# IntuitionMachines/volta

Hardware: AMD Instinct MI355X
Metric: image-text pairs/sec, ctrl_vilbert_base pretrain step (higher is better)
Workload: dtype bf16

## Files before the change

include/volta_hip.h:

```cpp
#ifndef VOLTA_HIP_H
#define VOLTA_HIP_H
#include <stddef.h>
#include <stdint.h>

#ifdef __cplusplus
extern "C" {
#endif

typedef void* vk_stream_t;

int vk_version(void);
const char* vk_device_arch(void);
const char* vk_last_error(void);

typedef struct vk_dropout {
    const uint64_t* seed;
    uint32_t site;
    uint32_t threshold;
    float scale;
} vk_dropout;

int vk_set_seed(uint64_t* seed_dev, uint64_t seed, vk_stream_t s);

int vk_cast_f32_bf16(const float* src, void* dst, int64_t n, vk_stream_t s);
// ... 256 lines not shown
int vk_nce_negatives(vk_dropout rng, int B, int R, int32_t* out, vk_stream_t s);

enum { VK_TASK_BCE_SCALED = 0, VK_TASK_BCE_MEAN = 1, VK_TASK_BCE_REGIONS = 2, VK_TASK_CE_OPTIONS = 3 };
typedef struct vk_task_loss_args {
    const float* logits;
    const void* target;
    const int64_t* mask;
    void* work;
    float* out;
    int32_t* row_argmax;
    int32_t kind, groups, n, ld;
} vk_task_loss_args;
int64_t vk_task_loss_work_bytes(int groups);
int vk_task_loss_fwd(const vk_task_loss_args* a, vk_stream_t s);
int vk_task_loss_bwd(const vk_task_loss_args* a, const float* gscale, void* dlogits, vk_stream_t s);

int vk_mask_prep(const int64_t* mask, float* out, int n, vk_stream_t s);

#define VK_CHUNK_SKIP 255
int vk_grad_norm_workspace_floats(void);
int vk_grad_norm_clip(const float* g, int64_t n, float pre_scale, float max_norm, float* partial, float* out, vk_stream_t s);
int vk_grad_norm_clip_masked(const float* g, int64_t n, const uint8_t* chunk_class, float pre_scale, float max_norm, float* partial, float* out, vk_stream_t s);
int vk_grad_sqnorm_chunks(const float* g, int64_t chunk0, int64_t nchunks, const uint8_t* chunk_class, float* sums, vk_stream_t s);
int vk_grad_norm_from_chunks(float* sums, int64_t total_chunks, float pre_scale, float max_norm, float* out, vk_stream_t s);
typedef struct vk_adamw_args {
    float* p;
    const float* g;
    float* m;
    float* v;
    void* shadow;
    const uint8_t* chunk_class;
    const float* clip;
    int64_t n;
    float cls_lr_mult[8];
    float cls_wd[8];
    float lr, beta1, beta2, eps, step_mult, grad_scale;
} vk_adamw_args;
int vk_adamw_step(const vk_adamw_args* a, vk_stream_t s);
int vk_adamw_step_on(const vk_adamw_args* a, int ncus, vk_stream_t s);
typedef struct vk_adamw_tensor {
    float* p;
    const float* g;
    float* m;
    float* v;
    int64_t numel;
    int32_t cls;
// ... 23 lines not shown
int vk_radam_step_list(const vk_radam_args* a, const vk_adamw_tensor* list, int n, int64_t max_numel, vk_stream_t s);
int vk_axpy_f32(float* y, const float* x, float alpha, int64_t n, vk_stream_t s);
int vk_sum_slabs_f32(float* dst, const float* src, int64_t slab_stride, int nslabs, int64_t n, vk_stream_t s);
int vk_sum_slabs_bf16(void* dst, const float* src, int64_t slab_stride, int nslabs, int64_t n, const int32_t* dyn_rows, int row_len, vk_stream_t s);
int vk_memset_async(void* p, int value, int64_t bytes, vk_stream_t s);
int vk_hold_cus(int nwg, int usec, int whole_cu, vk_stream_t s);
int vk_gate_wait(const uint64_t* flag, const uint64_t* stamp, int timeout_us, int32_t* err, vk_stream_t s);
int vk_bump_u64(uint64_t* word, vk_stream_t s);
int vk_store_u64(uint64_t* word, uint64_t value, vk_stream_t s);
int vk_gate_value(const uint64_t* flag, uint64_t want, int timeout_us, int32_t* err, vk_stream_t s);
int vk_comm_standin(const void* src, void* dst, int64_t bytes, int nwg, int min_usec, uint64_t* stamps, vk_stream_t s);
int vk_gemm_reserve_cus(int n);
#define VK_TAIL_MAX_JOBS 16
typedef struct vk_tail_job {
    float* dst;
    float* dst2;
    const float* src;
    const float* src2;
    int64_t stride;
    int64_t n;
    int32_t kind, count;
    int32_t accumulate;
    int32_t block_start;
} vk_tail_job;
int vk_side_tail(const vk_tail_job* jobs, int njobs, vk_stream_t s);

int vk_mul_bf16(const void* a, const void* b, void* out, int64_t n, const int32_t* dyn_rows, int row_len, vk_stream_t s);

enum {
    VK_OP_GEMM = 1,
    VK_OP_LN_FWD, VK_OP_LN_BWD,
    VK_OP_ATTN_FWD,
    VK_OP_ATTN_BWD,
    VK_OP_EMBED_FWD, VK_OP_EMBED_BWD, VK_OP_XENT_FWD,
    VK_OP_XENT_BWD,
    VK_OP_KL_FWD, VK_OP_KL_BWD,
    VK_OP_GENERIC,
    VK_OP_SIDE_BEGIN, VK_OP_SIDE_END, VK_OP_WAIT_SIDE, VK_OP_JOIN,
    VK_OP_LN_FINALIZE,
    VK_OP_GEMM_FP8,
    VK_OP_GEMM_CHAIN
};
enum {
    VK_FN_CAST = 1, VK_FN_MEMSET, VK_FN_LOC_FWD, VK_FN_LOC_BWD, VK_FN_ADD_DROPOUT, VK_FN_COLSUM, VK_FN_SELECT,
    VK_FN_GATHER, VK_FN_SCATTER_ADD, VK_FN_LOSS_FINAL, VK_FN_POOL_FWD, VK_FN_POOL_BWD, VK_FN_MASK_PREP, VK_FN_MUL,
    VK_FN_VLBERT_PREP, VK_FN_VLBERT_MASKGRAD, VK_FN_ROWGROUP_SUM, VK_FN_RELU_BWD, VK_FN_COPY, VK_FN_SUM_SLABS, VK_FN_SUM_SLABS_BF16,
// ... 103 lines not shown
```

volta_amd/_lib.py:

```python
import ctypes as C
import os

import torch

_HERE = os.path.dirname(os.path.abspath(__file__))
LIB_PATH = os.path.join(_HERE, "libvolta_hip_%s.so" % os.environ["VK_LIB"] if os.environ.get("VK_LIB") else "libvolta_hip.so")
GEMM_PERSISTENT, GEMM_ONE_TILE_PER_WG, GEMM_SOFT_START = 0x1000, 0x2000, 0x4000


class VoltaHipError(RuntimeError):
    pass


if not os.path.exists(LIB_PATH):
    raise ImportError(
        "volta_amd: %s not found. The HIP kernels are the product; there is no fallback path. "
        "Build with `make -C volta_amd/csrc` (hipcc --offload-arch=gfx950)." % LIB_PATH)

lib = C.CDLL(LIB_PATH)

c_p = C.c_void_p
i32 = C.c_int32
CHUNK_SKIP = 255

# ... 112 lines not shown
class RadamArgs(C.Structure):
    _fields_ = [("p", c_p), ("g", c_p), ("m", c_p), ("v", c_p), ("shadow", c_p), ("chunk_class", c_p), ("clip", c_p),
                ("n", C.c_int64), ("cls_decay", C.c_float * RADAM_CLASSES), ("cls_step", C.c_float * RADAM_CLASSES),
                ("cls_rect", i32 * RADAM_CLASSES), ("beta1", C.c_float), ("beta2", C.c_float), ("one_minus_beta1", C.c_float),
                ("one_minus_beta2", C.c_float), ("eps", C.c_float), ("grad_scale", C.c_float)]


class GradSeedArgs(C.Structure):
    _fields_ = [("src", c_p), ("stride_b", C.c_int64), ("stride_l", C.c_int64), ("dst", c_p), ("y", c_p), ("B", i32), ("L", i32), ("H", i32),
                ("row0", i32), ("ld", i32), ("ldy", i32), ("accumulate", i32), ("reserved_", i32)]


PAIR_MAX_SEGS = 8


class PairGatherArgs(C.Structure):
    _fields_ = [("src", c_p * PAIR_MAX_SEGS), ("dst", c_p * PAIR_MAX_SEGS), ("bytes", C.c_int64 * PAIR_MAX_SEGS), ("side", i32 * PAIR_MAX_SEGS),
                ("cap_idx", c_p), ("img_idx", c_p), ("n_items", C.c_int64 * 2), ("nseg", i32), ("npairs", i32), ("c0", i32), ("nc", i32),
                ("i0", i32), ("ni", i32)]


class TailJob(C.Structure):
    _fields_ = [("dst", c_p), ("dst2", c_p), ("src", c_p), ("src2", c_p), ("stride", C.c_int64), ("n", C.c_int64), ("kind", i32), ("count", i32),
                ("accumulate", i32), ("block_start", i32)]


TAIL_MAX_JOBS = 16


class GenericArgs(C.Structure):
    _fields_ = [("fn", i32), ("p", c_p * 6), ("n", C.c_int64 * 6), ("f", C.c_float * 2), ("drop", Dropout)]


class Op(C.Structure):
    _fields_ = [("kind", i32), ("i0", i32), ("i1", i32), ("i2", i32), ("a", c_p), ("b", c_p), ("c", c_p)]


(OP_GEMM, OP_LN_FWD, OP_LN_BWD, OP_ATTN_FWD, OP_ATTN_BWD, OP_EMBED_FWD, OP_EMBED_BWD, OP_XENT_FWD, OP_XENT_BWD,
 OP_KL_FWD, OP_KL_BWD, OP_GENERIC, OP_SIDE_BEGIN, OP_SIDE_END, OP_WAIT_SIDE, OP_JOIN, OP_LN_FINALIZE, OP_GEMM_FP8, OP_GEMM_CHAIN) = range(1, 20)
(FN_CAST, FN_MEMSET, FN_LOC_FWD, FN_LOC_BWD, FN_ADD_DROPOUT, FN_COLSUM, FN_SELECT, FN_GATHER, FN_SCATTER_ADD,
 FN_LOSS_FINAL, FN_POOL_FWD, FN_POOL_BWD, FN_MASK_PREP, FN_MUL, FN_VLBERT_PREP, FN_VLBERT_MASKGRAD, FN_ROWGROUP_SUM,
 FN_RELU_BWD, FN_COPY, FN_SUM_SLABS, FN_SUM_SLABS_BF16, FN_SIDE_TAIL, FN_QUANT_ROWS, FN_CAST_FP8, FN_VIS_LOSS_FWD, FN_VIS_LOSS_BWD,
 FN_NCE_NEG, FN_TEXT_END_ROWS, FN_VLBERT_OBJ_IDS, FN_VLBERT_POSITIONS, FN_HOLD, FN_GATE, FN_BUMP, FN_GRAD_SEED) = range(1, 35)


class AttnArgs(C.Structure):
    _fields_ = [("q", c_p * 2), ("k", c_p * 2), ("v", c_p * 2), ("ld", i32 * 2), ("L", i32 * 2), ("mask", c_p * 2),
# ... 78 lines not shown
_sig("vk_vlbert_positions", C.c_int, c_p, C.c_int, C.c_int, C.c_int, c_p, c_p, c_p)
_sig("vk_vis_loss_fwd", C.c_int, C.POINTER(VisLossArgs), c_p)
_sig("vk_vis_loss_bwd", C.c_int, C.POINTER(VisLossArgs), c_p, C.c_int, c_p, c_p)
_sig("vk_task_loss_work_bytes", C.c_int64, C.c_int)
_sig("vk_task_loss_fwd", C.c_int, C.POINTER(TaskLossArgs), c_p)
_sig("vk_task_loss_bwd", C.c_int, C.POINTER(TaskLossArgs), c_p, c_p, c_p)
_sig("vk_nce_negatives", C.c_int, Dropout, C.c_int, C.c_int, c_p, c_p)
_sig("vk_pool_mul_bwd", C.c_int, c_p, C.c_int, c_p, c_p, c_p, c_p, C.c_int, C.c_int, Dropout, c_p)
_sig("vk_mask_prep", C.c_int, c_p, c_p, C.c_int, c_p)
_sig("vk_mul_bf16", C.c_int, c_p, c_p, c_p, C.c_int64, c_p, C.c_int, c_p)
_sig("vk_grad_norm_workspace_floats", C.c_int)
_sig("vk_grad_norm_clip", C.c_int, c_p, C.c_int64, C.c_float, C.c_float, c_p, c_p, c_p)
_sig("vk_adamw_step", C.c_int, C.POINTER(AdamwArgs), c_p)
_sig("vk_adamw_step_on", C.c_int, C.POINTER(AdamwArgs), C.c_int, c_p)
_sig("vk_grad_norm_clip_masked", C.c_int, c_p, C.c_int64, c_p, C.c_float, C.c_float, c_p, c_p, c_p)
_sig("vk_adamw_step_list", C.c_int, C.POINTER(AdamwArgs), c_p, C.c_int, C.c_int64, c_p)
_sig("vk_grad_sqnorm_list", C.c_int, c_p, C.c_int, C.c_int64, c_p, c_p, c_p)
_sig("vk_grad_sqnorm_list_work_floats", C.c_int)
_sig("vk_grad_seed", C.c_int, C.POINTER(GradSeedArgs), c_p)
_sig("vk_pair_gather", C.c_int, C.POINTER(PairGatherArgs), c_p)
_sig("vk_radam_step", C.c_int, C.POINTER(RadamArgs), c_p)
_sig("vk_radam_step_list", C.c_int, C.POINTER(RadamArgs), c_p, C.c_int, C.c_int64, c_p)
_sig("vk_grad_sqnorm_chunks", C.c_int, c_p, C.c_int64, C.c_int64, c_p, c_p, c_p)
_sig("vk_grad_norm_from_chunks", C.c_int, c_p, C.c_int64, C.c_float, C.c_float, c_p, c_p)
_sig("vk_axpy_f32", C.c_int, c_p, c_p, C.c_float, C.c_int64, c_p)
_sig("vk_sum_slabs_f32", C.c_int, c_p, c_p, C.c_int64, C.c_int, C.c_int64, c_p)
_sig("vk_sum_slabs_bf16", C.c_int, c_p, c_p, C.c_int64, C.c_int, C.c_int64, c_p, C.c_int, c_p)
_sig("vk_memset_async", C.c_int, c_p, C.c_int, C.c_int64, c_p)
_sig("vk_hold_cus", C.c_int, C.c_int, C.c_int, C.c_int, c_p)
_sig("vk_gate_wait", C.c_int, c_p, c_p, C.c_int, c_p, c_p)
_sig("vk_bump_u64", C.c_int, c_p, c_p)
_sig("vk_store_u64", C.c_int, c_p, C.c_uint64, c_p)
_sig("vk_gate_value", C.c_int, c_p, C.c_uint64, C.c_int, c_p, c_p)
_sig("vk_comm_standin", C.c_int, c_p, c_p, C.c_int64, C.c_int, C.c_int, c_p, c_p)
_sig("vk_gemm_reserve_cus", C.c_int, C.c_int)
_sig("vk_side_tail", C.c_int, C.POINTER(TailJob), C.c_int, c_p)
_sig("vk_run_ops", C.c_int, C.POINTER(Op), C.c_int, c_p)
_sig("vk_run_ops_timed", C.c_int, C.POINTER(Op), C.c_int, c_p, C.POINTER(C.c_float))
_sig("vk_ln_bwd_finalize", C.c_int, C.POINTER(LnBwdArgs), c_p)
_sig("vk_ln_fwd_pair", C.c_int, C.POINTER(LnArgs), C.POINTER(LnArgs), c_p)
_sig("vk_ln_bwd_pair", C.c_int, C.POINTER(LnBwdArgs), C.POINTER(LnBwdArgs), c_p)
_sig("vk_concap_batch", C.c_int, C.POINTER(ConcapArgs), c_p)
_sig("vk_side_join", C.c_int, c_p)
_sig("vk_side_join_from", C.c_int, c_p, c_p)
_sig("vk_side_enable", None, C.c_int)
_sig("vk_side_stream", c_p, c_p)

EXPORTS = ["vk_version", "vk_device_arch", "vk_last_error", "vk_set_seed", "vk_cast_f32_bf16", "vk_gemm_grouped", "vk_gemm_grouped_ex", "vk_gemm_chain", "vk_gemm_split_workspace_bytes", "vk_gemm_fp8_grouped", "vk_quant_rows_fp8", "vk_cast_bf16_fp8",
           "vk_ln_fwd", "vk_ln_fwd_pair", "vk_ln_bwd_partial_rows", "vk_ln_bwd", "vk_ln_bwd_pair", "vk_ln_bwd_finalize", "vk_gated_attn_fwd", "vk_gated_attn_bwd", "vk_gated_attn_lds_bytes",
           "vk_embed_sum_fwd", "vk_embed_sum_bwd", "vk_embed_bwd_workspace_bytes", "vk_rows32", "vk_loc_linear_fwd", "vk_loc_linear_bwd",
           "vk_add_dropout", "vk_colsum_bf16", "vk_vlbert_prep_fwd", "vk_vlbert_maskgrad", "vk_rowgroup_sum_bf16",
           "vk_relu_bwd_bf16", "vk_copy_async", "vk_select_rows", "vk_gather_rows", "vk_scatter_rows_add", "vk_xent_fwd",
           "vk_xent_bwd", "vk_kl_fwd", "vk_kl_bwd", "vk_loss_finalize", "vk_pool_mul_fwd", "vk_pool_mul_bwd",
           "vk_pool_fuse_fwd", "vk_pool_fuse_bwd", "vk_text_end_rows", "vk_vlbert_obj_ids", "vk_vlbert_positions", "vk_vis_loss_fwd", "vk_vis_loss_bwd", "vk_nce_negatives", "vk_task_loss_work_bytes", "vk_task_loss_fwd", "vk_task_loss_bwd",
           "vk_mask_prep", "vk_mul_bf16", "vk_grad_norm_workspace_floats", "vk_grad_norm_clip", "vk_grad_norm_clip_masked", "vk_grad_sqnorm_chunks", "vk_grad_norm_from_chunks", "vk_adamw_step", "vk_adamw_step_on", "vk_adamw_step_list", "vk_grad_sqnorm_list", "vk_grad_sqnorm_list_work_floats", "vk_grad_seed", "vk_pair_gather", "vk_radam_step", "vk_radam_step_list",
           "vk_axpy_f32", "vk_sum_slabs_f32", "vk_sum_slabs_bf16", "vk_memset_async", "vk_hold_cus", "vk_gate_wait", "vk_bump_u64", "vk_store_u64", "vk_gate_value", "vk_comm_standin", "vk_gemm_reserve_cus", "vk_side_tail", "vk_run_ops", "vk_run_ops_timed", "vk_side_join", "vk_side_join_from", "vk_side_stream", "vk_side_enable", "vk_concap_batch",
           "vk_lmdb_open", "vk_lmdb_close", "vk_lmdb_entries", "vk_lmdb_first", "vk_lmdb_next", "vk_lmdb_get", "vk_concap_record_decode", "vk_concap_records_decode", "vk_b64_decode",
           "vk_wordpiece_open", "vk_wordpiece_close", "vk_wordpiece_vocab_size", "vk_wordpiece_token_id", "vk_wordpiece_encode", "vk_wordpiece_encode_batch"]


def check(rc):
    if rc != 0:
        raise VoltaHipError(lib.vk_last_error().decode())


def stream_ptr():
    return C.c_void_p(torch.cuda.current_stream().cuda_stream)


def ptr(t):
    return C.c_void_p(t.data_ptr()) if t is not None else None
```

volta_amd/csrc/optim.hip:

```cpp
#include "common.h"
#include "../../include/volta_hip.h"
#include "util.h"

namespace vk {

constexpr int NORM_BLOCKS = 1024;

__global__ __launch_bounds__(256) void sqnorm_partial_kernel(const float* g, size_t n4, float* partial, const uint8_t* chunk_class) {
    __shared__ float sh[4];
    float s = 0.f;
    for (size_t i = (size_t)blockIdx.x * 256 + threadIdx.x; i < n4; i += (size_t)gridDim.x * 256) {
        if (chunk_class && chunk_class[i >> 8] == VK_CHUNK_SKIP) continue;
        const f32x4 v = *(const f32x4*)(g + i * 4);
        s += v[0] * v[0] + v[1] * v[1] + v[2] * v[2] + v[3] * v[3];
    }
    s = wave_sum(s);
    if ((threadIdx.x & 63) == 0) sh[threadIdx.x >> 6] = s;
    __syncthreads();
    if (threadIdx.x == 0) partial[blockIdx.x] = sh[0] + sh[1] + sh[2] + sh[3];
}
__global__ __launch_bounds__(256) void sqnorm_final_kernel(const float* partial, int nblk, float pre_scale, float max_norm, float* out) {
    __shared__ double sh[4];
    double s = 0.0;
    for (int i = threadIdx.x; i < nblk; i += 256) s += (double)partial[i];
    for (int o = 32; o > 0; o >>= 1) s += __shfl_xor(s, o, 64);
    if ((threadIdx.x & 63) == 0) sh[threadIdx.x >> 6] = s;
    __syncthreads();
    if (threadIdx.x == 0) {
        const float norm = (float)sqrt(sh[0] + sh[1] + sh[2] + sh[3]) * pre_scale;
        out[0] = norm;
        float coef = 1.f;
        if (max_norm > 0.f) { coef = max_norm / (norm + 1e-6f); if (coef > 1.f) coef = 1.f; }
        out[1] = coef;
    }
}

__global__ __launch_bounds__(256) void sqnorm_chunks_kernel(const float* g, size_t chunk0, size_t nchunks, const uint8_t* chunk_class, float* sums) {
    const size_t c = (size_t)blockIdx.x * 4 + (threadIdx.x >> 6);
    if (c >= nchunks) return;
    const size_t chunk = chunk0 + c;
    const int lane = threadIdx.x & 63;
    float s = 0.f;
    if (!(chunk_class && chunk_class[chunk] == VK_CHUNK_SKIP)) {
        const float* p = g + chunk * 1024;
#pragma unroll
        for (int k = 0; k < 4; ++k) {
            const f32x4 v = __builtin_nontemporal_load((const f32x4*)(p + (k * 64 + lane) * 4));
            s += v[0] * v[0] + v[1] * v[1] + v[2] * v[2] + v[3] * v[3];
        }
    }
    s = wave_sum(s);
    if (lane == 0) sums[chunk] = s;
}
constexpr int SQ_GROUPS = 128;
__global__ __launch_bounds__(256) void sqnorm_groups_kernel(const float* sums, size_t n, double* group) {
    __shared__ double sh[4];
    const size_t per = (n + SQ_GROUPS - 1) / SQ_GROUPS, lo = (size_t)blockIdx.x * per, hi = lo + per < n ? lo + per : n;
    double s = 0.0;
    for (size_t i = lo + threadIdx.x; i < hi; i += 256) s += (double)sums[i];
    for (int o = 32; o > 0; o >>= 1) s += __shfl_xor(s, o, 64);
    if ((threadIdx.x & 63) == 0) sh[threadIdx.x >> 6] = s;
    __syncthreads();
    if (threadIdx.x == 0) group[blockIdx.x] = (sh[0] + sh[1]) + (sh[2] + sh[3]);
}
__global__ __launch_bounds__(64) void sqnorm_from_groups_kernel(const double* group, float pre_scale, float max_norm, float* out) {
    double s = group[threadIdx.x] + group[threadIdx.x + 64];
    for (int o = 32; o > 0; o >>= 1) s += __shfl_xor(s, o, 64);
    if (threadIdx.x == 0) {
        const float norm = (float)sqrt(s) * pre_scale;
        out[0] = norm;
        float coef = 1.f;
        if (max_norm > 0.f) { coef = max_norm / (norm + 1e-6f); if (coef > 1.f) coef = 1.f; }
        out[1] = coef;
    }
// ... 162 lines not shown
        f32x4 a = *(const f32x4*)(src + i * 4);
        for (int s = 1; s < nslabs; ++s) {
            const f32x4 b = *(const f32x4*)(src + (size_t)s * stride + i * 4);
#pragma unroll
            for (int r = 0; r < 4; ++r) a[r] += b[r];
        }
        *(u32x2*)(dst + i * 4) = u32x2{pack2bf(a[0], a[1]), pack2bf(a[2], a[3])};
    }
}

struct TailJobs { vk_tail_job j[VK_TAIL_MAX_JOBS]; int32_t njobs; };

__global__ __launch_bounds__(256) void side_tail_kernel(const TailJobs t) {
    __shared__ float red[16][17];
    int ji = 0;
#pragma unroll
    for (int i = 1; i < VK_TAIL_MAX_JOBS; ++i)
        if (i < t.njobs && (int)blockIdx.x >= t.j[i].block_start) ji = i;
    const vk_tail_job& J = t.j[ji];
    const int blk = (int)blockIdx.x - J.block_start;
    if (J.kind == 0) {
        const size_t n4 = (size_t)J.n >> 2;
        const size_t i = (size_t)blk * 256 + threadIdx.x;
        if (i < n4) {
            f32x4 a = __builtin_nontemporal_load((const f32x4*)(J.src + i * 4));
            for (int s = 1; s < J.count; ++s) {
                const f32x4 b = __builtin_nontemporal_load((const f32x4*)(J.src + (size_t)s * J.stride + i * 4));
#pragma unroll
                for (int r = 0; r < 4; ++r) a[r] += b[r];
            }
            __builtin_nontemporal_store(a, (f32x4*)(J.dst + i * 4));
        }
        if (blk == 0 && threadIdx.x < (J.n & 3)) {
            const size_t k = n4 * 4 + threadIdx.x;
            float a = 0.f;
            for (int s = 0; s < J.count; ++s) a += J.src[(size_t)s * J.stride + k];
            J.dst[k] = a;
        }
    } else {
        const int H = (int)J.n, tx = threadIdx.x & 15, ty = threadIdx.x >> 4;
        const int i = blk * 16 + tx;
        float s = 0.f;
        if (i < 2 * H) {
            for (int b = ty; b < J.count; b += 16) s += J.src[(size_t)b * 2 * H + i];
            if (J.src2)
                for (int b = ty; b < (int)J.stride; b += 16) s += J.src2[(size_t)b * 2 * H + i];
        }
        red[ty][tx] = s;
        __syncthreads();
        if (ty == 0 && i < 2 * H) {
#pragma unroll
            for (int k = 1; k < 16; ++k) s += red[k][tx];
            float* o = i < H ? J.dst + i : J.dst2 + (i - H);
            *o = J.accumulate ? *o + s : s;
        }
    }
}

}

using namespace vk;

extern "C" int vk_side_tail(const vk_tail_job* jobs, int njobs, vk_stream_t s) {
    if (njobs <= 0) return 0;
    if (njobs > VK_TAIL_MAX_JOBS) return set_error("vk_side_tail: %d jobs (max %d)", njobs, VK_TAIL_MAX_JOBS);
    TailJobs t;
    t.njobs = njobs;
    int total = 0;
    for (int i = 0; i < njobs; ++i) {
        t.j[i] = jobs[i];
        vk_tail_job& J = t.j[i];
        int nb;
        if (J.kind == 0) {
            if ((J.stride & 3) || ((uintptr_t)J.dst & 15) || ((uintptr_t)J.src & 15)) return set_error("vk_side_tail: slab job %d needs 16-byte alignment", i);
            nb = (int)((J.n / 4 + 255) / 256);
            if (nb < 1) nb = 1;
        } else if (J.kind == 1) {
            nb = (int)((2 * J.n + 15) / 16);
        } else return set_error("vk_side_tail: unknown job kind %d", J.kind);
        if (J.n <= 0 || J.count <= 0) nb = 0;
        J.block_start = total;
        total += nb;
    }
    if (total == 0) return 0;
    hipLaunchKernelGGL(side_tail_kernel, dim3((unsigned)total), dim3(256), 0, (hipStream_t)s, t);
    return check_launch("vk_side_tail");
}

extern "C" int vk_sum_slabs_bf16(void* dst, const float* src, int64_t slab_stride, int nslabs, int64_t n, const int32_t* dyn_rows, int row_len, vk_stream_t s) {
    if (n <= 0 || nslabs <= 0) return 0;
    if ((slab_stride & 3) || (n & 3) || (row_len & 3)) return set_error("vk_sum_slabs_bf16: lengths must be multiples of 4");
    int64_t blocks = (n / 4 + 255) / 256;
    if (blocks > 2048) blocks = 2048;
    hipLaunchKernelGGL(sum_slabs_bf16_kernel, dim3((unsigned)blocks), dim3(256), 0, (hipStream_t)s, (uint16_t*)dst, src, (size_t)slab_stride, nslabs, (size_t)n, dyn_rows, row_len);
    return check_launch("vk_sum_slabs_bf16");
}

extern "C" int vk_sum_slabs_f32(float* dst, const float* src, int64_t slab_stride, int nslabs, int64_t n, vk_stream_t s) {
    if (n <= 0 || nslabs <= 0) return 0;
    if ((slab_stride & 3) || ((uintptr_t)dst & 15) || ((uintptr_t)src & 15)) return set_error("vk_sum_slabs_f32: 16-byte alignment required");
    int64_t blocks = (n / 4 + 255) / 256;
    if (blocks > 2048) blocks = 2048;
    if (blocks < 1) blocks = 1;
    hipLaunchKernelGGL(sum_slabs_kernel, dim3((unsigned)blocks), dim3(256), 0, (hipStream_t)s, dst, src, (size_t)slab_stride, nslabs, (size_t)n);
    return check_launch("vk_sum_slabs_f32");
}

extern "C" int vk_grad_norm_workspace_floats(void) { return NORM_BLOCKS; }

extern "C" int vk_grad_norm_clip_masked(const float* g, int64_t n, const uint8_t* chunk_class, float pre_scale, float max_norm, float* partial, float* out, vk_stream_t s) {
    if (n % 4 || ((uintptr_t)g & 15)) return set_error("vk_grad_norm_clip: n %% 4 == 0 and 16-byte alignment required");
    if (chunk_class && (n % 1024)) return set_error("vk_grad_norm_clip_masked: a chunk mask needs an arena of whole 1024-element chunks");
    hipStream_t st = (hipStream_t)s;
    hipLaunchKernelGGL(sqnorm_partial_kernel, dim3(NORM_BLOCKS), dim3(256), 0, st, g, (size_t)(n / 4), partial, chunk_class);
    hipLaunchKernelGGL(sqnorm_final_kernel, dim3(1), dim3(256), 0, st, partial, NORM_BLOCKS, pre_scale, max_norm, out);
    return check_launch("vk_grad_norm_clip");
}

extern "C" int vk_grad_sqnorm_chunks(const float* g, int64_t chunk0, int64_t nchunks, const uint8_t* chunk_class, float* sums, vk_stream_t s) {
    if (chunk0 < 0 || nchunks < 0 || ((uintptr_t)g & 15)) return set_error("vk_grad_sqnorm_chunks: bad range or alignment");
    if (nchunks == 0) return 0;
    hipLaunchKernelGGL(sqnorm_chunks_kernel, dim3((unsigned)((nchunks + 3) / 4)), dim3(256), 0, (hipStream_t)s, g, (size_t)chunk0, (size_t)nchunks, chunk_class, sums);
    return check_launch("vk_grad_sqnorm_chunks");
}

extern "C" int vk_grad_norm_from_chunks(float* sums, int64_t total_chunks, float pre_scale, float max_norm, float* out, vk_stream_t s) {
    if (total_chunks <= 0) return set_error("vk_grad_norm_from_chunks: no chunks");
    if (((uintptr_t)(sums + total_chunks)) & 7) return set_error("vk_grad_norm_from_chunks: total_chunks must be even (the group sums follow the chunk sums as doubles)");
    double* group = (double*)(sums + total_chunks);
    hipLaunchKernelGGL(sqnorm_groups_kernel, dim3(SQ_GROUPS), dim3(256), 0, (hipStream_t)s, sums, (size_t)total_chunks, group);
    hipLaunchKernelGGL(sqnorm_from_groups_kernel, dim3(1), dim3(64), 0, (hipStream_t)s, (const double*)group, pre_scale, max_norm, out);
    return check_launch("vk_grad_norm_from_chunks");
}

extern "C" int vk_grad_norm_clip(const float* g, int64_t n, float pre_scale, float max_norm, float* partial, float* out, vk_stream_t s) {
    return vk_grad_norm_clip_masked(g, n, nullptr, pre_scale, max_norm, partial, out, s);
}

extern "C" int vk_adamw_step(const vk_adamw_args* a, vk_stream_t s) {
    if (a->n % 1024) return set_error("vk_adamw_step: arena length must be a multiple of 1024 elements");
    if (a->n == 0) return 0;
    hipLaunchKernelGGL(adamw_kernel, dim3((unsigned)(a->n / 1024)), dim3(256), 0, (hipStream_t)s, *a);
    return check_launch("vk_adamw_step");
}

extern "C" int vk_adamw_step_on(const vk_adamw_args* a, int ncus, vk_stream_t s) {
// ... 46 lines not shown
```

volta_amd/engine.py:

```python
import ctypes as C
import math
import os

import torch

from . import _lib as L
from ._lib import check, ptr
from .modules import sublayer_schedule

CHUNK = 1024
VIS_TARGET_WIDTH = {"0": 1601, "1": 2048, "2": 2048, "3": 1600, "4": 400, "5": 2048, "6": 1601}
NO_DECAY = ("bias", "LayerNorm.bias", "LayerNorm.weight")


def _round_up(x, m):
    return (x + m - 1) // m * m


class ParamArena:

    def __init__(self, model, device, prefix=""):
        named = [(prefix + n, p) for n, p in model.named_parameters()]
        byname = dict(named)
        slots, seen = [], set()
        for name, p in named:
            if name in seen:
# ... 15 lines not shown
            start = off
            for g in group:
                self.offset[g] = off
                self.shape[g] = tuple(byname[g].shape)
                off += byname[g].numel()
            off = _round_up(off, CHUNK)
            nd = any(k in group[0] for k in NO_DECAY)
            assert all(any(k in g for k in NO_DECAY) == nd for g in group)
            classes += [1 if nd else 0] * ((off - start) // CHUNK)
        self.total = off
        self.device = device
        self.master = torch.zeros(self.total, dtype=torch.float32, device=device)
        self.shadow = torch.zeros(self.total, dtype=torch.bfloat16, device=device)
        self.grad = torch.zeros(self.total, dtype=torch.float32, device=device)
        self.chunk_class = torch.tensor(classes, dtype=torch.uint8, device=device)
        self.names = [n for n, _ in named]
        self.params = byname
        with torch.no_grad():
            for name, p in named:
                v = self.view(name)
                v.copy_(p.data.to(device=device, dtype=torch.float32))
                p.data = v
                p.grad = None
        self.shadow_version = -1
        self.weights_epoch = 0
        self.fp8_sites = {}
        self.fp8_epoch = -1

    def view(self, name, which="master"):
        buf = getattr(self, which)
        o = self.offset[name]
        n = 1
        for d in self.shape[name]:
            n *= d
        return buf[o:o + n].view(self.shape[name])

    def param_list(self):
        if getattr(self, "_plist", None) is None or len(self._plist) != len(self.params):
            self._plist = list(self.params.items())
        return self._plist

    def grad_views(self):
        if getattr(self, "_gviews", None) is None or len(self._gviews) != len(self.params):
            self._gviews = [self.view(n, "grad") for n in self.params]
        return self._gviews

    def span(self, names, which, shape):
        buf = getattr(self, which)
        o = self.offset[names[0]]
        n = 1
        for d in shape:
            n *= d
        for a, b in zip(names[:-1], names[1:]):
            assert self.offset[b] == self.offset[a] + int(torch.tensor(self.shape[a]).prod())
        return buf[o:o + n].view(shape)

    def intact(self):
        return all(p.data_ptr() == self.master.data_ptr() + 4 * self.offset[n] for n, p in self.params.items())
# ... 20 lines not shown
            Kp = _round_up(K, 128)
            self.fp8_sites[key] = (w, torch.zeros(N, Kp, dtype=torch.uint8, device=self.device), torch.ones(N, dtype=torch.float32, device=self.device))
            self.fp8_epoch = -1
        return self.fp8_sites[key][1:]

    def refresh_fp8(self):
        if self.fp8_epoch == self.weights_epoch:
            return
        for w, q, sc in self.fp8_sites.values():
            N, K = w.shape
            check(L.lib.vk_quant_rows_fp8(ptr(w), 1, w.stride(0), ptr(q), q.stride(0), ptr(sc), N, K, None, L.stream_ptr()))
        self.fp8_epoch = self.weights_epoch

    def invalidate_shadow(self):
        self.shadow_version = -1

    def sync_optimizer(self):
        pend = getattr(self, "opt_pending", None)
        if pend:
            cur = torch.cuda.current_stream()
            for ev in pend[1]:
                cur.wait_event(ev)
            self.opt_pending = None


class Plan:
    def __init__(self):
        self.ops, self.keep = [], []
        self.c_ops = None
        self.timing = None

    def add(self, kind, a, i0=0, i1=0, i2=0, b=None, c=None):
        self.ops.append((kind, i0, i1, i2, a, b, c))

    def freeze(self):
        arr = (L.Op * max(1, len(self.ops)))()
        for i, (kind, i0, i1, i2, a, b, c) in enumerate(self.ops):
            arr[i] = L.Op(kind, i0, i1, i2, _addr(a), _addr(b), _addr(c))
        self.c_ops = arr
        return self

    def run(self, start=0, end=None):
        end = len(self.ops) if end is None else end
        if end > start:
            base = C.cast(C.byref(self.c_ops, start * C.sizeof(L.Op)), C.POINTER(L.Op))
            if self.timing is not None:
# ... 69 lines not shown
        if self.wide and fp8:
            raise NotImplementedError("the fp8 projection path covers the single-width (ctrl_*) geometry")
        if self.wide and cfg.image_embeddings != "vilbert":
            raise NotImplementedError("different stream widths are built for the ViLBERT embeddings (config/vilbert_base.json)")
        if cfg.hidden_act != "gelu" or cfg.v_hidden_act != "gelu":
            raise NotImplementedError("engine supports gelu activations (every reference config)")
        if cfg.fusion_method not in ("mul", "sum", "text", "vl-bert_vqa", "none"):
            raise ValueError("Invalid fusion method: %s" % cfg.fusion_method)
        self.unused_params = set()
        if T + Rv > 512:
            raise NotImplementedError("more than 512 keys per query row (%d text + %d vision rows)" % (T, Rv))
        self.H, self.I, self.nh = H, cfg.intermediate_size, cfg.num_attention_heads
        self.st = [Stream(T, B, H), Stream(Rv, B, Hv)]
        self.R = Rv - (1 if cfg.add_global_imgfeat is not None else 0)
        self.bufs = {}
        self.keep = []
        self.fwd, self.bwd = Plan(), Plan()
        self.bwd_groups = []
        self.site = 0
        self.seed = torch.zeros(1, dtype=torch.int64, device=dev)
        self.inputs = {}
        self.taps = {}
        self.grad_seeds = {}
        self._build()

    def buf(self, name, shape, dtype=torch.bfloat16, zero=False):
        assert name not in self.bufs, name
        t = (torch.zeros if zero else torch.empty)(shape, dtype=dtype, device=self.dev)
        self.bufs[name] = t
        return t

    def embed_ws(self, eb, tag):
        n = L.lib.vk_embed_bwd_workspace_bytes(eb.M, eb.H, eb.V, eb.P, int(bool(eb.pos_ids) and bool(eb.dpos)))
        eb.work = _addr(self.tmp("embed_ws_" + tag, (max(n, 1),), torch.uint8))
        return eb

    def tmp(self, name, shape, dtype=torch.bfloat16):
        name += getattr(self, "_aside", "")
        if name not in self.bufs:
            self.bufs[name] = torch.empty(shape, dtype=dtype, device=self.dev)
        t = self.bufs[name]
        assert tuple(t.shape) == tuple(shape) and t.dtype == dtype, (name, t.shape, shape)
        return t

    def drop(self, p):
        site = self.site
        self.site += 1
# ... 983 lines not shown
            if len(chunks) == 1:
                dY, X, rows, lda, ldb = chunks[0]
                probs.append(self.prob(dY, X, gW, Mo, No, rows, lda, ldb, No, bias_grad=gB))
                continue
            stride = _round_up(Mo * No + Mo, 4)
            slab = self._slab(len(chunks) * stride)
            for i, (dY, X, rows, lda, ldb) in enumerate(chunks):
                base = slab[i * stride:]
                probs.append(self.prob(dY, X, base, Mo, No, rows, lda, ldb, No, bias_grad=base[Mo * No:]))
            reduces.append((gW, slab, stride, len(chunks), Mo * No))
            reduces.append((gB, slab[Mo * No:], stride, len(chunks), Mo))
        assert len(probs) <= 32, "too many wgrad problems in one group"
        gate = self._gate_words() if self.side_gate else None
        b.append((L.OP_SIDE_BEGIN, 1 if gate is not None else 0, 0, 0, None, None, None))
        if gate is not None:
            self._n_gate = getattr(self, "_n_gate", 0) + 1
            assert self._n_gate < gate.numel()
            flag = gate.data_ptr() + 8 * self._n_gate
            b.append((L.OP_GENERIC, 0, 0, 0, self.generic(L.FN_GATE, p=(flag, gate.data_ptr(), self.bufs["gate_err"]), n=(1000000,)), None, None))
            self._gate_flag = (flag, gate.data_ptr())
        if self.side_delay_us > 0:
            b.append((L.OP_GENERIC, 0, 0, 0, self.generic(L.FN_HOLD, n=(1, self.side_delay_us, 0)), None, None))
        self.gemm(b, L.TN, L.EPI_F32, probs)
        jobs = [L.TailJob(_addr(dst), None, _addr(src), None, stride, n, 0, ns, 0, 0) for dst, src, stride, ns, n in reduces]
        by_dst = {}
        for a in getattr(self, "_deferred_ln", []):
            by_dst.setdefault(a.dgamma, []).append(a)
        for group in by_dst.values():
            assert len(group) <= 2 and not (group[0].accumulate & 1) and all(g.accumulate & 1 for g in group[1:]), "unexpected LayerNorm sharing"
            a, b2 = group[0], (group[1] if len(group) > 1 else None)
            jobs.append(L.TailJob(a.dgamma, a.dbeta, a.partial, b2.partial if b2 else None, L.lib.vk_ln_bwd_partial_rows(b2.M) if b2 else 0, a.H, 1,
                                  L.lib.vk_ln_bwd_partial_rows(a.M), 0, 0))
        self._deferred_ln = []
        for i in range(0, len(jobs), L.TAIL_MAX_JOBS):
            chunk = jobs[i:i + L.TAIL_MAX_JOBS]
            arr = self.k((L.TailJob * len(chunk))(*chunk))
            b.append((L.OP_GENERIC, 0, 0, 0, self.generic(L.FN_SIDE_TAIL, p=(arr,), n=(len(chunk),)), None, None))
        b.append((L.OP_SIDE_END, self.sub_k % 8, 0, 0, None, None, None))
        self._slab_cursor = 0

    def _gate_words(self):
        if "gate_words" not in self.bufs:
            self.bufs["gate_words"] = torch.zeros(128, dtype=torch.int64, device=self.dev)
            self.bufs["gate_words"][1:] = -1
            self.bufs["gate_err"] = torch.zeros(1, dtype=torch.int32, device=self.dev)
            g = self.bufs["gate_words"]
            self.bwd_pro.append((L.OP_GENERIC, 0, 0, 0, self.generic(L.FN_BUMP, p=(g,)), None, None))
            self.bwd_pro.append((L.OP_SIDE_BEGIN, 0, 0, 0, None, None, None))
            self.bwd_pro.append((L.OP_SIDE_END, 13, 0, 0, None, None, None))
        return self.bufs["gate_words"]

    def retire_on(self, probs):
        gf = getattr(self, "_gate_flag", None)
        if gf is not None:
            probs[0].retire_flag, probs[0].retire_stamp = gf
            self._gate_flag = None
        return probs

    def _slab(self, n):
        cap = 48 * 3072 * 768
        ws = self.tmp("wgrad_slabs", (cap,), torch.float32)
        cur = getattr(self, "_slab_cursor", 0)
# ... 453 lines not shown
```

volta_amd/modeling.py:

```python
import logging
import os

import torch
from torch import nn

from . import modules as M
from .config import BertConfig

logger = logging.getLogger(__name__)


class ArenaParameters:

    __slots__ = ("vk_model", "started", "_it")

    def __init__(self, model, it):
        self.vk_model, self.started, self._it = model, False, it

    def __iter__(self):
        return self

    def __next__(self):
        self.started = True
        return next(self._it)
# ... 414 lines not shown
        eng.arena.refresh_shadow()
        if eng.fp8:
            eng.arena.sync_optimizer()
            eng.arena.refresh_fp8()
        eng.bind_inputs(tensors)
        if self._seed_base is None:
            self.__dict__["_seed_base"] = int(torch.initial_seed())
        eng.prepare_step(self._seed_base + self._step)
        self.__dict__["_step"] += 1
        eng.run_forward()
        self.__dict__["_last"] = (eng, tensors)
        return getattr(eng, "losses", None)

    def _engine_backward(self, g_lm, g_img, g_nsp):
        eng, tensors = self._last
        state = self._backward_begin(eng)
        torch.cat([g_lm.reshape(1), g_img.reshape(1), g_nsp.reshape(1)], out=eng.gout)
        self._backward_run(eng, state)

    def _backward_begin(self, eng, absent=()):
        arena = eng.arena
        from .optimization import flush_clip
        flush_clip(arena)
        skip = getattr(self, "_torch_param_prefixes", ())
        unused = eng.unused_params
        pairs = [((n, p), g) for (n, p), g in zip(arena.param_list(), arena.grad_views())
                 if p.requires_grad and not (skip and n.startswith(skip)) and n not in unused and n not in absent]
        params, gviews = [x[0] for x in pairs], [x[1] for x in pairs]
        n_have = sum(p.grad is not None for _, p in params)
        accumulate = n_have == len(params)
        if n_have and not accumulate:
            raise RuntimeError("volta_amd: some parameters carry a .grad and some do not; zero_grad() all of them")
        old = None
        if accumulate:
            if not all(p.grad is g or p.grad.data_ptr() == g.data_ptr() for (_, p), g in zip(params, gviews)):
                raise RuntimeError("volta_amd: .grad tensors were replaced by foreign tensors; call zero_grad(set_to_none=True)")
            old = arena.grad.clone()
        return params, gviews, accumulate, old

    def _backward_run(self, eng, state):
        params, gviews, accumulate, old = state
        arena = eng.arena
        skip = getattr(self, "_torch_param_prefixes", ())
        if skip:
            keep = [(g, g.clone()) for (n, _), g in zip(arena.param_list(), arena.grad_views()) if n.startswith(skip)] if accumulate else []
        ddp = self.__dict__.get("_ddp")
        if ddp is not None:
            ddp.run_backward(eng)
        else:
            eng.bwd.run()
        if accumulate:
            from . import _lib as L
            L.check(L.lib.vk_axpy_f32(L.ptr(arena.grad), L.ptr(old), 1.0, arena.total, L.stream_ptr()))
            if skip:
                for g, saved in keep:
                    g.copy_(saved)
        else:
            for (_, p), g in zip(params, gviews):
                p.grad = g

    def forward(self, input_ids, image_feat, image_loc, token_type_ids=None, attention_mask=None,
                image_attention_mask=None, masked_lm_labels=None, image_label=None, image_cls=None, obj_labels=None,
                obj_confs=None, attr_labels=None, attr_confs=None, image_attrs=None, next_sentence_label=None,
                output_all_attention_masks=False):
        if masked_lm_labels is None and next_sentence_label is None:
            return self._scores(input_ids, image_feat, image_loc, token_type_ids, attention_mask, image_attention_mask, image_label,
                                output_all_attention_masks)
        if masked_lm_labels is None or image_label is None:
            raise NotImplementedError("the pre-training step needs masked_lm_labels and image_label")
        tensors, B, T, Rv = self._prep_inputs(input_ids, image_feat, image_loc, token_type_ids, attention_mask,
                                              image_attention_mask, masked_lm_labels, image_label, image_cls, next_sentence_label,
                                              obj_labels, obj_confs, attr_labels, attr_confs)
        if torch.is_grad_enabled() and any(p.requires_grad for p in self.parameters()):
            self.materialize()
            anchor = next(p for p in self.parameters() if p.requires_grad)
            return _PretrainStep.apply(self, anchor, tensors)
        losses = self._engine_forward(tensors)
        return losses[0:1].clone(), losses[1:2].clone(), losses[2:3].clone()

    def _scores(self, input_ids, image_feat, image_loc, token_type_ids, attention_mask, image_attention_mask, image_label, output_all_attention_masks=False):
        from . import _lib as L, ops
        if image_label is not None and bool((image_label == 1).any()):
# ... 344 lines not shown
```

volta_amd/optimization.py:

```python
import ctypes as C
import math
import os

import numpy as np
import torch
import weakref

from torch.optim import Optimizer
from torch.optim.lr_scheduler import LambdaLR

from . import _lib as L


def _split_params(params, labels=None):
    labels = labels or ["parameter %d" % i for i in range(len(params))]
    owners, foreign = {}, []
    for p, lab in zip(params, labels):
        o = getattr(p, "_vk_owner", None)
        if o is not None:
            owners.setdefault(id(o), (o, lab))
        else:
            foreign.append((p, lab))
    if len(owners) > 1:
        (_, a), (_, b) = list(owners.values())[:2]
# ... 717 lines not shown
            raise RuntimeError("clip_grad_norm_: the gradient of %s is not attached to the engine's arena (run backward first)" % n)
        have.append(n)
    if not have and not any(p.grad is not None for p in foreign):
        raise RuntimeError("clip_grad_norm_: gradients are not attached to the engine's arena (run backward first)")
    flive = [p for p in foreign if p.grad is not None]
    if flive and _red_mode(model) == "zero1":
        raise NotImplementedError("clip_grad_norm_: data-parallel mode 'zero1' with parameters outside the model's arena")
    mask = None
    if len(have) != len(plist):
        cache = arena.__dict__.setdefault("_clip_masks", {})
        key = tuple(have)
        if key not in cache:
            if len(cache) > 16:
                cache.clear()
            _check_shared_chunks(arena, set(have), "part of the norm")
            cc = torch.full((arena.total // 1024,), L.CHUNK_SKIP, dtype=torch.uint8)
            for n in have:
                c0, c1 = _chunks_of(arena, n)
                cc[c0:c1] = 0
            cache[key] = cc.to(arena.device)
        mask = cache[key]
    nchunks = arena.total // 1024
    npad = nchunks + (nchunks & 1)
    if not hasattr(arena, "norm_chunks"):
        arena.norm_chunks = torch.zeros(npad + 256, device=arena.device)
    sums = arena.norm_chunks[:npad]
    if flive:
        nf = len(flive)
        npad = nchunks + nf + ((nchunks + nf) & 1)
        buf = arena.__dict__.get("norm_slots")
        if buf is None or buf.numel() < npad + 256:
            buf = arena.__dict__["norm_slots"] = torch.zeros(npad + 256, device=arena.device)
        sums = buf[:npad]
        sums[nchunks + nf:].zero_()
        ents = [(p, p.grad, None, None, 0) for p in flive]
        for p in flive:
            if p.grad.dtype != torch.float32 or not p.grad.is_contiguous() or p.grad.device != arena.device:
                raise RuntimeError("clip_grad_norm_: the gradient of a tensor outside the arena must be a contiguous float32 tensor on %s" % arena.device)
        flist, fmax = _tensor_list(ents, arena.device)
        work = torch.empty(nf * L.lib.vk_grad_sqnorm_list_work_floats(), device=arena.device)
        L.check(L.lib.vk_grad_sqnorm_list(L.ptr(flist), nf, fmax, L.ptr(work), L.ptr(sums[nchunks:]), L.stream_ptr()))
    out = torch.empty(2, device=arena.device)
    ddp = getattr(model, "_ddp", None)
    red = getattr(ddp, "reducer", None)
    if red is not None and red.mode == "zero1" and (red.sharded or red.replicated):
        sums.zero_()
        mine = [(lo + red.rank * s, lo + (red.rank + 1) * s) for lo, hi, s in red.sharded] + (list(red.replicated) if red.rank == 0 else [])
        for lo, hi in mine:
            L.check(L.lib.vk_grad_sqnorm_chunks(L.ptr(arena.grad), lo // 1024, (hi - lo) // 1024, L.ptr(mask), L.ptr(sums), L.stream_ptr()))
        torch.distributed.all_reduce(sums, group=red.pg)
    else:
        L.check(L.lib.vk_grad_sqnorm_chunks(L.ptr(arena.grad), 0, nchunks, L.ptr(mask), L.ptr(sums), L.stream_ptr()))
    L.check(L.lib.vk_grad_norm_from_chunks(L.ptr(sums), npad, pre_scale, float(max_norm), L.ptr(out), L.stream_ptr()))
    names = frozenset(have + [("foreign", id(p)) for p in flive])
    if defer_to_optimizer is None:
        opt = getattr(arena, "_vk_adamw", None)
        opt = opt() if opt is not None else None
        defer_to_optimizer = opt is not None and opt._fused is not None and opt._fused["arena"] is arena and opt._grad_names() == names
    arena.pending_clip = (out, names, [p.grad for p in flive]) if flive else (out, names)
    if not defer_to_optimizer:
        flush_clip(arena)
    return out[0]


def _red_mode(model):
    red = getattr(getattr(model, "_ddp", None), "reducer", None)
    return red.mode if red is not None and (red.sharded or red.replicated) else None


def _clip_foreign_only(params, max_norm, pre_scale):
    live = [p for p in params if p.grad is not None]
    if not live:
        raise RuntimeError("clip_grad_norm_: no parameter carries a gradient")
# ... 13 lines not shown
```

Measured before the change: 15290.

## Fuse gradient chunk squared-norm into backward slab-reduce tail jobs

Slab-reduce tail jobs that write a chunk-aligned gradient region now also compute per-chunk squared sums into the arena's norm buffer. Gradient clipping then only rereads the uncovered chunks through a new list-driven kernel, skipping a full pass over the gradient arena. Reuse is keyed on the grad tensor version, and the summation order is pinned so the norm stays bitwise identical. The cost is a block reduction added to the tail jobs plus extra bookkeeping, and a stale-stamp risk if the gradients are touched outside the tracked paths.

```diff
diff --git a/include/volta_hip.h b/include/volta_hip.h
--- a/include/volta_hip.h
+++ b/include/volta_hip.h
@@ -302,6 +302,7 @@
 int vk_grad_norm_clip(const float* g, int64_t n, float pre_scale, float max_norm, float* partial, float* out, vk_stream_t s);
 int vk_grad_norm_clip_masked(const float* g, int64_t n, const uint8_t* chunk_class, float pre_scale, float max_norm, float* partial, float* out, vk_stream_t s);
 int vk_grad_sqnorm_chunks(const float* g, int64_t chunk0, int64_t nchunks, const uint8_t* chunk_class, float* sums, vk_stream_t s);
+int vk_grad_sqnorm_chunk_list(const float* g, const int32_t* list, int64_t nchunks, const uint8_t* chunk_class, float* sums, vk_stream_t s);
 int vk_grad_norm_from_chunks(float* sums, int64_t total_chunks, float pre_scale, float max_norm, float* out, vk_stream_t s);
 typedef struct vk_adamw_args {
     float* p;
@@ -371,6 +372,8 @@
     int32_t kind, count;
     int32_t accumulate;
     int32_t block_start;
+    float* sums;
+    int64_t chunk0;
 } vk_tail_job;
 int vk_side_tail(const vk_tail_job* jobs, int njobs, vk_stream_t s);
 
diff --git a/volta_amd/_lib.py b/volta_amd/_lib.py
--- a/volta_amd/_lib.py
+++ b/volta_amd/_lib.py
@@ -158,7 +158,7 @@
 
 class TailJob(C.Structure):
     _fields_ = [("dst", c_p), ("dst2", c_p), ("src", c_p), ("src2", c_p), ("stride", C.c_int64), ("n", C.c_int64), ("kind", i32), ("count", i32),
-                ("accumulate", i32), ("block_start", i32)]
+                ("accumulate", i32), ("block_start", i32), ("sums", c_p), ("chunk0", C.c_int64)]
 
 
 TAIL_MAX_JOBS = 16
@@ -283,6 +283,7 @@
 _sig("vk_radam_step", C.c_int, C.POINTER(RadamArgs), c_p)
 _sig("vk_radam_step_list", C.c_int, C.POINTER(RadamArgs), c_p, C.c_int, C.c_int64, c_p)
 _sig("vk_grad_sqnorm_chunks", C.c_int, c_p, C.c_int64, C.c_int64, c_p, c_p, c_p)
+_sig("vk_grad_sqnorm_chunk_list", C.c_int, c_p, c_p, C.c_int64, c_p, c_p, c_p)
 _sig("vk_grad_norm_from_chunks", C.c_int, c_p, C.c_int64, C.c_float, C.c_float, c_p, c_p)
 _sig("vk_axpy_f32", C.c_int, c_p, c_p, C.c_float, C.c_int64, c_p)
 _sig("vk_sum_slabs_f32", C.c_int, c_p, c_p, C.c_int64, C.c_int, C.c_int64, c_p)
@@ -314,7 +315,7 @@
            "vk_relu_bwd_bf16", "vk_copy_async", "vk_select_rows", "vk_gather_rows", "vk_scatter_rows_add", "vk_xent_fwd",
            "vk_xent_bwd", "vk_kl_fwd", "vk_kl_bwd", "vk_loss_finalize", "vk_pool_mul_fwd", "vk_pool_mul_bwd",
            "vk_pool_fuse_fwd", "vk_pool_fuse_bwd", "vk_text_end_rows", "vk_vlbert_obj_ids", "vk_vlbert_positions", "vk_vis_loss_fwd", "vk_vis_loss_bwd", "vk_nce_negatives", "vk_task_loss_work_bytes", "vk_task_loss_fwd", "vk_task_loss_bwd",
-           "vk_mask_prep", "vk_mul_bf16", "vk_grad_norm_workspace_floats", "vk_grad_norm_clip", "vk_grad_norm_clip_masked", "vk_grad_sqnorm_chunks", "vk_grad_norm_from_chunks", "vk_adamw_step", "vk_adamw_step_on", "vk_adamw_step_list", "vk_grad_sqnorm_list", "vk_grad_sqnorm_list_work_floats", "vk_grad_seed", "vk_pair_gather", "vk_radam_step", "vk_radam_step_list",
+           "vk_mask_prep", "vk_mul_bf16", "vk_grad_norm_workspace_floats", "vk_grad_norm_clip", "vk_grad_norm_clip_masked", "vk_grad_sqnorm_chunks", "vk_grad_sqnorm_chunk_list", "vk_grad_norm_from_chunks", "vk_adamw_step", "vk_adamw_step_on", "vk_adamw_step_list", "vk_grad_sqnorm_list", "vk_grad_sqnorm_list_work_floats", "vk_grad_seed", "vk_pair_gather", "vk_radam_step", "vk_radam_step_list",
            "vk_axpy_f32", "vk_sum_slabs_f32", "vk_sum_slabs_bf16", "vk_memset_async", "vk_hold_cus", "vk_gate_wait", "vk_bump_u64", "vk_store_u64", "vk_gate_value", "vk_comm_standin", "vk_gemm_reserve_cus", "vk_side_tail", "vk_run_ops", "vk_run_ops_timed", "vk_side_join", "vk_side_join_from", "vk_side_stream", "vk_side_enable", "vk_concap_batch",
            "vk_lmdb_open", "vk_lmdb_close", "vk_lmdb_entries", "vk_lmdb_first", "vk_lmdb_next", "vk_lmdb_get", "vk_concap_record_decode", "vk_concap_records_decode", "vk_b64_decode",
            "vk_wordpiece_open", "vk_wordpiece_close", "vk_wordpiece_vocab_size", "vk_wordpiece_token_id", "vk_wordpiece_encode", "vk_wordpiece_encode_batch"]
diff --git a/volta_amd/csrc/optim.hip b/volta_amd/csrc/optim.hip
--- a/volta_amd/csrc/optim.hip
+++ b/volta_amd/csrc/optim.hip
@@ -35,21 +35,27 @@
     }
 }
 
-__global__ __launch_bounds__(256) void sqnorm_chunks_kernel(const float* g, size_t chunk0, size_t nchunks, const uint8_t* chunk_class, float* sums) {
+__device__ __forceinline__ float sq4(const f32x4 v) {
+#pragma clang fp contract(off)
+    return __builtin_fmaf(v[3], v[3], __builtin_fmaf(v[2], v[2], __builtin_fmaf(v[1], v[1], v[0] * v[0])));
+}
+__device__ __forceinline__ float chunk_sqsum(float q0, float q1, float q2, float q3) {
+#pragma clang fp contract(off)
+    return wave_sum(((q0 + q1) + q2) + q3);
+}
+
+__global__ __launch_bounds__(256) void sqnorm_chunks_kernel(const float* g, size_t chunk0, size_t nchunks, const int32_t* list, const uint8_t* chunk_class, float* sums) {
     const size_t c = (size_t)blockIdx.x * 4 + (threadIdx.x >> 6);
     if (c >= nchunks) return;
-    const size_t chunk = chunk0 + c;
+    const size_t chunk = list ? (size_t)list[c] : chunk0 + c;
     const int lane = threadIdx.x & 63;
-    float s = 0.f;
+    float q[4] = {0.f, 0.f, 0.f, 0.f};
     if (!(chunk_class && chunk_class[chunk] == VK_CHUNK_SKIP)) {
         const float* p = g + chunk * 1024;
 #pragma unroll
-        for (int k = 0; k < 4; ++k) {
-            const f32x4 v = __builtin_nontemporal_load((const f32x4*)(p + (k * 64 + lane) * 4));
-            s += v[0] * v[0] + v[1] * v[1] + v[2] * v[2] + v[3] * v[3];
-        }
-    }
-    s = wave_sum(s);
+        for (int k = 0; k < 4; ++k) q[k] = sq4(__builtin_nontemporal_load((const f32x4*)(p + (k * 64 + lane) * 4)));
+    }
+    const float s = chunk_sqsum(q[0], q[1], q[2], q[3]);
     if (lane == 0) sums[chunk] = s;
 }
 constexpr int SQ_GROUPS = 128;
@@ -258,14 +264,24 @@
     if (J.kind == 0) {
         const size_t n4 = (size_t)J.n >> 2;
         const size_t i = (size_t)blk * 256 + threadIdx.x;
+        f32x4 a = {0.f, 0.f, 0.f, 0.f};
         if (i < n4) {
-            f32x4 a = __builtin_nontemporal_load((const f32x4*)(J.src + i * 4));
+            a = __builtin_nontemporal_load((const f32x4*)(J.src + i * 4));
             for (int s = 1; s < J.count; ++s) {
                 const f32x4 b = __builtin_nontemporal_load((const f32x4*)(J.src + (size_t)s * J.stride + i * 4));
 #pragma unroll
                 for (int r = 0; r < 4; ++r) a[r] += b[r];
             }
             __builtin_nontemporal_store(a, (f32x4*)(J.dst + i * 4));
+        }
+        if (J.sums) {
+            float* ex = &red[0][0];
+            ex[threadIdx.x] = sq4(a);
+            __syncthreads();
+            if (threadIdx.x < 64) {
+                const float s = chunk_sqsum(ex[threadIdx.x], ex[64 + threadIdx.x], ex[128 + threadIdx.x], ex[192 + threadIdx.x]);
+                if (threadIdx.x == 0) J.sums[J.chunk0 + blk] = s;
+            }
         }
         if (blk == 0 && threadIdx.x < (J.n & 3)) {
             const size_t k = n4 * 4 + threadIdx.x;
@@ -309,9 +325,11 @@
         int nb;
         if (J.kind == 0) {
             if ((J.stride & 3) || ((uintptr_t)J.dst & 15) || ((uintptr_t)J.src & 15)) return set_error("vk_side_tail: slab job %d needs 16-byte alignment", i);
+            if (J.sums && ((J.n & 3) || J.chunk0 < 0)) return set_error("vk_side_tail: slab job %d emits chunk sums: n %% 4 == 0 and a chunk index >= 0 required", i);
             nb = (int)((J.n / 4 + 255) / 256);
             if (nb < 1) nb = 1;
         } else if (J.kind == 1) {
+            if (J.sums) return set_error("vk_side_tail: job %d: only slab jobs emit chunk sums", i);
             nb = (int)((2 * J.n + 15) / 16);
         } else return set_error("vk_side_tail: unknown job kind %d", J.kind);
         if (J.n <= 0 || J.count <= 0) nb = 0;
@@ -356,8 +374,15 @@
 extern "C" int vk_grad_sqnorm_chunks(const float* g, int64_t chunk0, int64_t nchunks, const uint8_t* chunk_class, float* sums, vk_stream_t s) {
     if (chunk0 < 0 || nchunks < 0 || ((uintptr_t)g & 15)) return set_error("vk_grad_sqnorm_chunks: bad range or alignment");
     if (nchunks == 0) return 0;
-    hipLaunchKernelGGL(sqnorm_chunks_kernel, dim3((unsigned)((nchunks + 3) / 4)), dim3(256), 0, (hipStream_t)s, g, (size_t)chunk0, (size_t)nchunks, chunk_class, sums);
+    hipLaunchKernelGGL(sqnorm_chunks_kernel, dim3((unsigned)((nchunks + 3) / 4)), dim3(256), 0, (hipStream_t)s, g, (size_t)chunk0, (size_t)nchunks, (const int32_t*)nullptr, chunk_class, sums);
     return check_launch("vk_grad_sqnorm_chunks");
+}
+
+extern "C" int vk_grad_sqnorm_chunk_list(const float* g, const int32_t* list, int64_t nchunks, const uint8_t* chunk_class, float* sums, vk_stream_t s) {
+    if (nchunks < 0 || ((uintptr_t)g & 15) || (nchunks > 0 && !list)) return set_error("vk_grad_sqnorm_chunk_list: bad list or alignment");
+    if (nchunks == 0) return 0;
+    hipLaunchKernelGGL(sqnorm_chunks_kernel, dim3((unsigned)((nchunks + 3) / 4)), dim3(256), 0, (hipStream_t)s, g, (size_t)0, (size_t)nchunks, list, chunk_class, sums);
+    return check_launch("vk_grad_sqnorm_chunk_list");
 }
 
 extern "C" int vk_grad_norm_from_chunks(float* sums, int64_t total_chunks, float pre_scale, float max_norm, float* out, vk_stream_t s) {
diff --git a/volta_amd/engine.py b/volta_amd/engine.py
--- a/volta_amd/engine.py
+++ b/volta_amd/engine.py
@@ -2,6 +2,7 @@
 import math
 import os
 
+import numpy as np
 import torch
 
 from . import _lib as L
@@ -63,6 +64,8 @@
                 v.copy_(p.data.to(device=device, dtype=torch.float32))
                 p.data = v
                 p.grad = None
+        self._spans = sorted((self.offset[n], byname[n].numel()) for n in byname)
+        self.norm_stamp = None
         self.shadow_version = -1
         self.weights_epoch = 0
         self.fp8_sites = {}
@@ -75,6 +78,16 @@
         for d in self.shape[name]:
             n *= d
         return buf[o:o + n].view(self.shape[name])
+
+    def norm_sums(self):
+        if not hasattr(self, "norm_chunks"):
+            nchunks = self.total // CHUNK
+            self.norm_chunks = torch.zeros(nchunks + (nchunks & 1) + 256, device=self.device)
+        return self.norm_chunks
+
+    def padding_behind(self, end):
+        hi = _round_up(end, CHUNK)
+        return not any(o < hi and o + n > end for o, n in self._spans)
 
     def param_list(self):
         if getattr(self, "_plist", None) is None or len(self._plist) != len(self.params):
@@ -141,6 +154,26 @@
             for ev in pend[1]:
                 cur.wait_event(ev)
             self.opt_pending = None
+
+
+class NormCover:
+
+    def __init__(self, arena, ranges):
+        nch = arena.total // CHUNK
+        cnt = np.zeros(nch, dtype=np.int32)
+        for c0, c1 in ranges:
+            assert 0 <= c0 < c1 <= nch, (c0, c1, nch)
+            cnt[c0:c1] += 1
+        cov = cnt == 1
+        self.covered, self.rest = _ranges(cov), _ranges(~cov)
+        rest = np.flatnonzero(~cov).astype(np.int32)
+        self.n_rest = int(rest.size)
+        self.rest_list = torch.from_numpy(rest).to(arena.device) if rest.size else None
+
+
+def _ranges(flags):
+    edges = np.flatnonzero(np.diff(np.concatenate(([0], flags.astype(np.int8), [0]))))
+    return [(int(a), int(b)) for a, b in zip(edges[0::2], edges[1::2])]
 
 
 class Plan:
@@ -256,7 +289,9 @@
         self.inputs = {}
         self.taps = {}
         self.grad_seeds = {}
+        self.norm_covered = []
         self._build()
+        self.norm_cover = NormCover(arena, self.norm_covered) if self.bwd.ops else None
 
     def buf(self, name, shape, dtype=torch.bfloat16, zero=False):
         assert name not in self.bufs, name
@@ -1286,7 +1321,7 @@
         if self.side_delay_us > 0:
             b.append((L.OP_GENERIC, 0, 0, 0, self.generic(L.FN_HOLD, n=(1, self.side_delay_us, 0)), None, None))
         self.gemm(b, L.TN, L.EPI_F32, probs)
-        jobs = [L.TailJob(_addr(dst), None, _addr(src), None, stride, n, 0, ns, 0, 0) for dst, src, stride, ns, n in reduces]
+        jobs = [self._tail_slab_job(dst, src, stride, ns, n) for dst, src, stride, ns, n in reduces]
         by_dst = {}
         for a in getattr(self, "_deferred_ln", []):
             by_dst.setdefault(a.dgamma, []).append(a)
@@ -1302,6 +1337,14 @@
             b.append((L.OP_GENERIC, 0, 0, 0, self.generic(L.FN_SIDE_TAIL, p=(arr,), n=(len(chunk),)), None, None))
         b.append((L.OP_SIDE_END, self.sub_k % 8, 0, 0, None, None, None))
         self._slab_cursor = 0
+
+    def _tail_slab_job(self, dst, src, stride, ns, n):
+        arena, sums, c0 = self.arena, None, -1
+        off = (dst.data_ptr() - arena.grad.data_ptr()) // 4
+        if 0 <= off and off + n <= arena.total and off % CHUNK == 0 and n % 4 == 0 and arena.padding_behind(off + n):
+            sums, c0 = arena.norm_sums().data_ptr(), off // CHUNK
+            self.norm_covered.append((c0, c0 + -(-n // CHUNK)))
+        return L.TailJob(_addr(dst), None, _addr(src), None, stride, n, 0, ns, 0, 0, sums, c0)
 
     def _gate_words(self):
         if "gate_words" not in self.bufs:
diff --git a/volta_amd/modeling.py b/volta_amd/modeling.py
--- a/volta_amd/modeling.py
+++ b/volta_amd/modeling.py
@@ -460,6 +460,7 @@
         arena = eng.arena
         from .optimization import flush_clip
         flush_clip(arena)
+        arena.norm_stamp = None
         skip = getattr(self, "_torch_param_prefixes", ())
         unused = eng.unused_params
         pairs = [((n, p), g) for (n, p), g in zip(arena.param_list(), arena.grad_views())
@@ -496,6 +497,8 @@
         else:
             for (_, p), g in zip(params, gviews):
                 p.grad = g
+            if ddp is None and not skip:
+                arena.norm_stamp = (eng.norm_cover, arena.grad._version)
 
     def forward(self, input_ids, image_feat, image_loc, token_type_ids=None, attention_mask=None,
                 image_attention_mask=None, masked_lm_labels=None, image_label=None, image_cls=None, obj_labels=None,
diff --git a/volta_amd/optimization.py b/volta_amd/optimization.py
--- a/volta_amd/optimization.py
+++ b/volta_amd/optimization.py
@@ -763,9 +763,11 @@
         mask = cache[key]
     nchunks = arena.total // 1024
     npad = nchunks + (nchunks & 1)
-    if not hasattr(arena, "norm_chunks"):
-        arena.norm_chunks = torch.zeros(npad + 256, device=arena.device)
-    sums = arena.norm_chunks[:npad]
+    sums = arena.norm_sums()[:npad]
+    stamp, arena.norm_stamp = getattr(arena, "norm_stamp", None), None
+    cover = None
+    if stamp is not None and mask is None and not flive and getattr(model, "_ddp", None) is None and stamp[0] is not None and stamp[1] == arena.grad._version:
+        cover = stamp[0]
     if flive:
         nf = len(flive)
         npad = nchunks + nf + ((nchunks + nf) & 1)
@@ -790,6 +792,9 @@
         for lo, hi in mine:
             L.check(L.lib.vk_grad_sqnorm_chunks(L.ptr(arena.grad), lo // 1024, (hi - lo) // 1024, L.ptr(mask), L.ptr(sums), L.stream_ptr()))
         torch.distributed.all_reduce(sums, group=red.pg)
+    elif cover is not None:
+        arena.norm_fast_clips = getattr(arena, "norm_fast_clips", 0) + 1
+        L.check(L.lib.vk_grad_sqnorm_chunk_list(L.ptr(arena.grad), L.ptr(cover.rest_list), cover.n_rest, None, L.ptr(sums), L.stream_ptr()))
     else:
         L.check(L.lib.vk_grad_sqnorm_chunks(L.ptr(arena.grad), 0, nchunks, L.ptr(mask), L.ptr(sums), L.stream_ptr()))
     L.check(L.lib.vk_grad_norm_from_chunks(L.ptr(sums), npad, pre_scale, float(max_norm), L.ptr(out), L.stream_ptr()))
```

After: 15290 (median of 2 runs). About the same (-0.0%).
